# jacke121/p265

Hardware: AMD Instinct MI355X
Metric: reconstructed CTUs/sec (1080p all-intra) + achieved HBM GB/s vs peak (higher is better)
Workload: dtype u8 samples / int16 coefficients (integer)

## Files before the change

p265_amd/csrc/p265r.hip:

```cpp
#include <hip/hip_runtime.h>

#include <algorithm>
#include <array>
#include <chrono>
#include <cstdio>
#include <cstdlib>
#include <ctime>
#include <cstring>
#include <new>
#include <string>
#include <vector>

#include "../../include/p265r.h"
#include "digest.h"
#include "export.h"
#include "export_host.h"
#include "intra.h"
#include "intra_prep.h"
#include "intra_rows.h"
#include "loopfilter.h"
#include "loopfilter16.h"
#include "sao16.h"
#include "residual.h"
#include "coef_expand.h"
// ... 805 lines not shown
    *h2d_bytes = b->h2d_bytes;
    return P265R_OK;
}

int p265r_batch_run(p265r_ctx* ctx, p265r_batch* b) {
    if (!ctx || !b) return P265R_EINVAL;
    HIP_TRY(hipSetDevice(ctx->device));
    hipStream_t s = b->stream;
    Geo g = ctx->geo;
    g.ragged = b->ragged ? 1 : 0;
    p265r_timings tm{};
    hipEvent_t ev[4] = {nullptr, nullptr, nullptr, nullptr};
    if (ctx->timing) {
        for (auto& e : ev) {
            if (!ctx->spare.empty()) { e = ctx->spare.back(); ctx->spare.pop_back(); }
            else HIP_TRY(hipEventCreate(&e));
        }
        HIP_TRY(hipEventRecord(ev[0], s));
    }
    const int bdl = g.bd[0], bdc = g.bd[1];
    const bool recon = !b->recon_input;
    const int skip = b->runs > 0 ? ctx->skip : 0;
    if (ctx->params.scaling_list_enabled && !ctx->d_sf && !b->recon_input) return P265R_ESTATE;
    const uint8_t* sf = ctx->params.scaling_list_enabled ? ctx->d_sf : nullptr;
    ++b->runs;
    ctx->lane_busy |= 1u << b->lane;
    const bool prep = recon && ctx->schedule == 1 && !(skip & 2);
    hipStream_t ps = s;
    const bool big = b->n_pics >= ctx->num_cus;
    const bool sao_aux = P265R_SAO_AUX && !P265R_PHASE_ORDER && !P265R_EARLY_RESIDUAL && ctx->pipeline > 1 && big && prep &&
                         !ctx->timing && ctx->fork_prep == 1 && (b->sao || b->dbk) && !(skip & 4);
    const int fork_prep = big && !sao_aux ? ctx->fork_prep : 0;
    const bool ordered = P265R_PHASE_ORDER && ctx->pipeline > 1 && prep && fork_prep == 1 && !ctx->timing;
    const bool early = !ordered && P265R_EARLY_RESIDUAL && prep && fork_prep == 1 && !ctx->timing && b->intra_done &&
                       !(skip & 1);
    hipEvent_t r_after = ordered ? (ctx->last_intra_valid ? ctx->last_intra_ev : nullptr) : (early ? b->intra_done : nullptr);
    if (ordered && ctx->order_r == 0) r_after = b->intra_done;
    hipStream_t rs = s;
    if ((ordered || early) && r_after) {
        const size_t li = (size_t)b->lane;
        if (ctx->aux2.size() <= li) { ctx->aux2.resize(li + 1, nullptr); ctx->join2_ev.resize(li + 1, nullptr); }
        if (!ctx->aux2[li]) {
            HIP_TRY(hipStreamCreateWithFlags(&ctx->aux2[li], hipStreamNonBlocking));
            HIP_TRY(hipEventCreateWithFlags(&ctx->join2_ev[li], hipEventDisableTiming));
        }
        rs = ctx->aux2[li];
        HIP_TRY(hipStreamWaitEvent(rs, r_after, 0));
        if (b->intra_done && r_after != b->intra_done) HIP_TRY(hipStreamWaitEvent(rs, b->intra_done, 0));
    }
    if (prep && fork_prep) {
        const size_t li = fork_prep == 2 ? 0 : (size_t)b->lane;
        if (ctx->aux.size() <= li) {
            ctx->aux.resize(li + 1, nullptr); ctx->fork_ev.resize(li + 1, nullptr); ctx->join_ev.resize(li + 1, nullptr);
        }
        if (!ctx->aux[li]) {
            if (ctx->stream_prio) {
                int least = 0, greatest = 0;
                HIP_TRY(hipDeviceGetStreamPriorityRange(&least, &greatest));
                HIP_TRY(hipStreamCreateWithPriority(&ctx->aux[li], hipStreamNonBlocking, least));
            } else {
                HIP_TRY(hipStreamCreateWithFlags(&ctx->aux[li], hipStreamNonBlocking));
            }
            HIP_TRY(hipEventCreateWithFlags(&ctx->fork_ev[li], hipEventDisableTiming));
            HIP_TRY(hipEventCreateWithFlags(&ctx->join_ev[li], hipEventDisableTiming));
        }
        ps = ctx->aux[li];
        if ((ordered || early) && r_after) {
            HIP_TRY(hipStreamWaitEvent(ps, r_after, 0));
            if (b->intra_done && r_after != b->intra_done) HIP_TRY(hipStreamWaitEvent(ps, b->intra_done, 0));
        } else {
            HIP_TRY(hipEventRecord(ctx->fork_ev[li], s));
            HIP_TRY(hipStreamWaitEvent(ps, ctx->fork_ev[li], 0));
        }
    }
    auto launch_prep = [&]() -> int {
        Geo gp = g;
        gp.tr_info = (2 * (long long)b->n_pics <= ctx->num_cus || ctx->row_waves == 16) ? 1 : 0;
        intra_prep_kernel<<<dim3(g.wc, g.hc, b->n_pics), 64, ctx->prep_lds, ps>>>(b->d_pics, gp, b->view);
        ++tm.residual_launches;
        if (ps != s) HIP_TRY(hipEventRecord(ctx->join_ev[fork_prep == 2 ? 0 : (size_t)b->lane], ps));
        return P265R_OK;
    };
    if (prep && !ctx->prep_last) { int rc = launch_prep(); if (rc) return rc; }
#define P265R_RES_LAUNCH(K, KSL, blocks, ...)                                                                     \
    do {                                                                                                          \
        if (sf) KSL<<<(blocks), 256, ctx->res_lds, rs>>>(__VA_ARGS__, sf);                                        \
        else K<<<(blocks), 256, ctx->res_lds, rs>>>(__VA_ARGS__, nullptr);                                        \
        ++tm.residual_launches;                                                                                   \
    } while (0)
    if (recon && !(skip & 1) && b->n_jobs[RC_DST4])
        P265R_RES_LAUNCH((residual4_kernel<true, false>), (residual4_kernel<true, true>), (b->n_jobs[RC_DST4] + 255) / 256,
                         b->d_pool, b->d_res, b->d_jobs[RC_DST4], b->n_jobs[RC_DST4], bdl, b->slab[RC_DST4]);
    if (recon && !(skip & 1) && b->n_jobs[RC_DCT4])
        P265R_RES_LAUNCH((residual4_kernel<false, false>), (residual4_kernel<false, true>), (b->n_jobs[RC_DCT4] + 255) / 256,
                         b->d_pool, b->d_res, b->d_jobs[RC_DCT4], b->n_jobs[RC_DCT4], bdc, b->slab[RC_DCT4]);
    if (recon && !(skip & 1) && b->n_jobs[RC_DCT8])
        P265R_RES_LAUNCH((residualN_kernel<3, false>), (residualN_kernel<3, true>), (b->n_jobs[RC_DCT8] + 31) / 32,
                         b->d_pool, b->d_res, b->d_jobs[RC_DCT8], b->n_jobs[RC_DCT8], bdl, bdc, b->slab[RC_DCT8]);
    if (recon && !(skip & 1) && b->n_jobs[RC_DCT16])
        P265R_RES_LAUNCH((residualN_kernel<4, false>), (residualN_kernel<4, true>), (b->n_jobs[RC_DCT16] + 15) / 16,
                         b->d_pool, b->d_res, b->d_jobs[RC_DCT16], b->n_jobs[RC_DCT16], bdl, bdc, b->slab[RC_DCT16]);
    if (recon && !(skip & 1) && b->n_jobs[RC_DCT32])
        P265R_RES_LAUNCH((residualN_kernel<5, false>), (residualN_kernel<5, true>), (b->n_jobs[RC_DCT32] + 7) / 8,
                         b->d_pool, b->d_res, b->d_jobs[RC_DCT32], b->n_jobs[RC_DCT32], bdl, bdc, b->slab[RC_DCT32]);
#undef P265R_RES_LAUNCH
    if (recon && !(skip & 1) && b->n_jobs[RC_TSKIP]) {
        residual_tskip_kernel<<<(b->n_jobs[RC_TSKIP] + 255) / 256, 256, 0, rs>>>(b->d_pool, b->d_res, b->d_jobs[RC_TSKIP], b->n_jobs[RC_TSKIP], bdl, bdc, sf);
        ++tm.residual_launches;
    }
    if (prep && ctx->prep_last) { int rc = launch_prep(); if (rc) return rc; }
    if (prep && ps != s) HIP_TRY(hipStreamWaitEvent(s, ctx->join_ev[fork_prep == 2 ? 0 : (size_t)b->lane], 0));
    if (rs != s) {
        HIP_TRY(hipEventRecord(ctx->join2_ev[(size_t)b->lane], rs));
        HIP_TRY(hipStreamWaitEvent(s, ctx->join2_ev[(size_t)b->lane], 0));
    }
    if (b->dbk) {
        if (g.pel16) dbk_map_kernel<uint16_t><<<dim3(ctx->n_ctus, b->n_pics), 64, 0, s>>>(b->d_pics, g);
        else dbk_map_kernel<uint8_t><<<dim3(ctx->n_ctus, b->n_pics), 64, 0, s>>>(b->d_pics, g);
        ++tm.residual_launches;
    }
    HIP_TRY(hipGetLastError());
    if (ctx->debug_sync) { fprintf(stderr, "[p265r] residual phase enqueued\n"); HIP_TRY(hipStreamSynchronize(s)); fprintf(stderr, "[p265r] residual phase done\n"); }
    if (ctx->timing) HIP_TRY(hipEventRecord(ev[1], s));
    if (recon && ctx->schedule == 1) {
        HIP_TRY(hipMemsetAsync(b->d_err + 64, 0, kRowCuSlots * 16 + (b->d_xg_prog ? sizeof(int) * 2 * ((size_t)g.hc + 1) * b->n_pics : 0), s));
        if (b->sao_pending) { HIP_TRY(hipStreamWaitEvent(s, b->sao_done, 0)); b->sao_pending = false; }
        if (ordered && ctx->last_lf_valid) HIP_TRY(hipStreamWaitEvent(s, ctx->last_lf_ev, 0));
        bool alone = ordered || (ctx->lane_busy & ~(1u << b->lane)) == 0u;
#ifdef P265R_ALONE_PIPE
        alone = alone && ctx->pipeline == 1;
#endif
        int rc = launch_rows(ctx, b, s, alone);
        if (rc) return rc;
        ++tm.intra_launches;
    }
    const int n_steps = (recon && ctx->schedule == 0) ? (g.wc - 1) + 2 * (g.hc - 1) + 1 : 0;
    for (int step = 0; step < n_steps; ++step) {
        const int d = step - (g.wc - 1);
        const int cy_min = d > 0 ? (d + 1) / 2 : 0;
        const int cy_max = std::min(g.hc - 1, step / 2);
        if (cy_max < cy_min) continue;
        dim3 grid(cy_max - cy_min + 1, b->n_pics);
        if (g.pel16) intra_step_kernel<uint16_t><<<grid, 64, 0, s>>>(b->d_pics, b->d_pool, b->d_res, g, step, cy_min);
        else intra_step_kernel<uint8_t><<<grid, 64, 0, s>>>(b->d_pics, b->d_pool, b->d_res, g, step, cy_min);
        ++tm.intra_launches;
    }
    HIP_TRY(hipGetLastError());
    if (recon) {
        if (!b->intra_done) HIP_TRY(hipEventCreateWithFlags(&b->intra_done, hipEventDisableTiming));
        HIP_TRY(hipEventRecord(b->intra_done, s));
        if (!ctx->last_intra_ev) HIP_TRY(hipEventCreateWithFlags(&ctx->last_intra_ev, hipEventDisableTiming));
        HIP_TRY(hipEventRecord(ctx->last_intra_ev, s));
        ctx->last_intra_valid = true;
    }
    if (ctx->debug_sync) { fprintf(stderr, "[p265r] intra phase enqueued\n"); HIP_TRY(hipStreamSynchronize(s)); fprintf(stderr, "[p265r] intra phase done\n"); }
    if (ctx->timing) HIP_TRY(hipEventRecord(ev[2], s));
    const hipStream_t lane_s = s;
    if (sao_aux) {
        const size_t li = (size_t)b->lane;
        if (ctx->aux.size() <= li) {
            ctx->aux.resize(li + 1, nullptr); ctx->fork_ev.resize(li + 1, nullptr); ctx->join_ev.resize(li + 1, nullptr);
        }
        if (!ctx->aux[li]) {
            HIP_TRY(hipStreamCreateWithFlags(&ctx->aux[li], hipStreamNonBlocking));
            HIP_TRY(hipEventCreateWithFlags(&ctx->fork_ev[li], hipEventDisableTiming));
            HIP_TRY(hipEventCreateWithFlags(&ctx->join_ev[li], hipEventDisableTiming));
        }
        if (!b->sao_done) HIP_TRY(hipEventCreateWithFlags(&b->sao_done, hipEventDisableTiming));
        s = ctx->aux[li];
        HIP_TRY(hipStreamWaitEvent(s, b->intra_done, 0));
    }
    if (!(skip & 4)) {
        int rc = launch_loop_filters(ctx, b, g, s, &tm.sao_launches);
        if (rc) return rc;
    }
    if (sao_aux) {
        HIP_TRY(hipEventRecord(b->sao_done, s));
        b->sao_pending = true;
        s = lane_s;
    }
    if (ordered) {
        if (!ctx->last_lf_ev) HIP_TRY(hipEventCreateWithFlags(&ctx->last_lf_ev, hipEventDisableTiming));
        HIP_TRY(hipEventRecord(ctx->last_lf_ev, s));
        ctx->last_lf_valid = true;
    }
    if (ctx->timing) {
        HIP_TRY(hipEventRecord(ev[3], s));
        p265r_ctx::Run run;
        for (int i = 0; i < 4; ++i) run.ev[i] = ev[i];
        run.counts = tm;
// ... 219 lines not shown
    (void)join_sao(b);
    if (ctx->pending == b) ctx->pending = nullptr;
    hipError_t e = b->stream ? hipStreamSynchronize(b->stream) : hipSuccess;
    if (b->intra_done) (void)hipEventDestroy(b->intra_done);
    if (b->sao_done) (void)hipEventDestroy(b->sao_done);
    if (b->d_dig) (void)hipFree(b->d_dig);
    for (void* p : b->exp_idx) (void)hipFree(p);
    if (b->mem) {
        if (!ctx->cache_mem || b->bytes > ctx->cache_bytes) {
            if (ctx->cache_mem) e = hipFree(ctx->cache_mem);
            ctx->cache_mem = b->mem;
            ctx->cache_bytes = b->bytes;
        } else {
            e = hipFree(b->mem);
        }
    }
    delete b;
    return e == hipSuccess ? P265R_OK : hip_fail(e, "hipFree");
}

int p265r_submit(p265r_ctx* ctx, const p265r_picture* pics, int n_pics) {
    if (!ctx) return P265R_EINVAL;
    if (ctx->pending) return P265R_ESTATE;
    p265r_batch* b = nullptr;
    int rc = p265r_batch_upload(ctx, pics, n_pics, &b);
    if (rc) return rc;
    rc = p265r_batch_run(ctx, b);
    if (rc) { p265r_batch_free(ctx, b); return rc; }
    ctx->pending = b;
    ctx->pending_pics.assign(pics, pics + n_pics);
    return P265R_OK;
}

int p265r_wait(p265r_ctx* ctx) {
    if (!ctx) return P265R_EINVAL;
    if (!ctx->pending) return P265R_ESTATE;
    p265r_batch* b = ctx->pending;
    int rc = p265r_batch_download(ctx, b, ctx->pending_pics.data(), (int)ctx->pending_pics.size());
    ctx->pending = nullptr;
    ctx->pending_pics.clear();
    int rc2 = p265r_batch_free(ctx, b);
    return rc ? rc : rc2;
}

int p265r_sync(p265r_ctx* ctx) {
    if (!ctx) return P265R_EINVAL;
    HIP_TRY(hipSetDevice(ctx->device));
    for (hipStream_t st : ctx->lanes) HIP_TRY(hipStreamSynchronize(st));
    for (hipStream_t st : ctx->aux) if (st) HIP_TRY(hipStreamSynchronize(st));
    for (hipStream_t st : ctx->aux2) if (st) HIP_TRY(hipStreamSynchronize(st));
    ctx->lane_busy = 0;
    return P265R_OK;
}

int p265r_set_pipeline(p265r_ctx* ctx, int depth) {
    if (!ctx || depth < 1 || depth > 16) return P265R_EINVAL;
    HIP_TRY(hipSetDevice(ctx->device));
    while ((int)ctx->lanes.size() < depth) {
        hipStream_t st = nullptr;
        HIP_TRY(lane_stream_create(ctx, &st));
        ctx->lanes.push_back(st);
    }
    ctx->pipeline = depth;
    ctx->next_lane = 0;
    return P265R_OK;
}

static const char* hwq_env() {
    const char* v = std::getenv("GPU_MAX_HW_QUEUES");
    return (v && std::strlen(v) < 8 && std::strspn(v, "0123456789") == std::strlen(v)) ? v : "default";
}

int p265r_describe(p265r_ctx* ctx, char* buf, int size) {
    if (!ctx || size < 0 || (size > 0 && !buf)) return P265R_EINVAL;
    const Geo& g = ctx->geo;
    char tmp[2048];
    const int n = snprintf(tmp, sizeof(tmp),
        "{\"schedule\": \"%s\", \"row_waves\": %d, \"row_waves_by_run\": \"%s\", \"lean\": %d, "
        "\"fair\": %d, \"quad\": %d, \"luma_lead\": %d, \"sao_rows\": %d, \"skip\": %d, \"debug_sync\": %d, "
        "\"pipeline\": %d, \"fork_prep\": %d, \"pipe_waves\": %d, \"hw_queues\": \"%s\", \"num_cus\": %d, \"diag_build\": %d, "
        "\"experiments_build\": %d, \"split\": %d, \"last_launch_split\": %d, \"xg\": %d, \"last_launch_xg\": %d, "
        "\"phase_order\": %d, \"early_residual\": %d, \"bit_depth\": %d, \"row_launches\": {\"w12\": %lld, \"w8\": %lld, \"w16_split\": %lld, \"xg\": %lld, \"other\": %lld}, "
        "\"sparse_expand\": \"%s\", \"sparse_expand_stream\": %d, \"last_sparse_expand_ms\": %.4f, "
        "\"env_overrides\": [%s]}",
        ctx->schedule ? "rows" : "steps", ctx->row_waves,
        ctx->row_waves ? "fixed" : (P265R_PHASE_ORDER
                                   ? "batches of >= 1 picture per CU in a pipelined context: W=12, one intra launch at a time "
                                     "(phase order); small batches (< 1 picture per CU: component split, W=16): side by side; "
                                     "otherwise W=12 while no other lane has a run enqueued since the API synchronised it, "
                                     "else pipe_waves"
                                   : "batches of <= CUs / (2 xg) pictures: every luma / chroma chain on xg workgroups of W=4 "
                                     "(cross-group rows, progress and lines in global memory); small batches (< 1 picture per "
                                     "CU: component split, W=16); otherwise W=12 while no other "
                                     "lane has a run enqueued since the API synchronised it, else pipe_waves (W=8, 80 VGPRs: "
                                     "the other lanes' residual / prep / SAO waves fit beside it)"),
        ctx->lean, g.fair, g.quad, ctx->luma_lead, ctx->sao_rows, ctx->skip, ctx->debug_sync ? 1 : 0,
        ctx->pipeline, ctx->fork_prep, ctx->pipe_waves, hwq_env(), ctx->num_cus,
#ifdef P265R_DEBUG_DIAG
        1,
#else
        0,
#endif
        P265R_EXPERIMENTS, ctx->split, ctx->last_split ? 1 : 0, ctx->xg, ctx->last_xg ? 1 : 0, P265R_PHASE_ORDER, P265R_EARLY_RESIDUAL,
        (int)ctx->params.bit_depth_luma, ctx->row_launches[0], ctx->row_launches[1], ctx->row_launches[2], ctx->row_launches[3], ctx->row_launches[4],
        P265R_EXPAND_SCATTER ? "memset + global scatter" : "lds tile", P265R_EXPAND_STREAM, ctx->last_expand_ms,
        ctx->describe.c_str());
    if (n < 0) return P265R_EINVAL;
    if (size > 0) {
        const int k = std::min(n, size - 1);
        std::memcpy(buf, tmp, (size_t)k);
        buf[k] = 0;
    }
    return n;
}

int p265r_set_scaling_factors(p265r_ctx* ctx, const uint8_t* factors, int n_bytes) {
    if (!ctx || !factors || n_bytes != P265R_SCALING_FACTOR_BYTES) return P265R_EINVAL;
    if (!ctx->params.scaling_list_enabled) return P265R_ESTATE;
    for (int i = 0; i < n_bytes; ++i)
        if (factors[i] == 0) return P265R_EINVAL;
    HIP_TRY(hipSetDevice(ctx->device));
    if (int rc = p265r_sync(ctx)) return rc;
    if (!ctx->d_sf) HIP_TRY(hipMalloc(reinterpret_cast<void**>(&ctx->d_sf), P265R_SCALING_FACTOR_BYTES));
    HIP_TRY(hipMemcpy(ctx->d_sf, factors, P265R_SCALING_FACTOR_BYTES, hipMemcpyHostToDevice));
    return P265R_OK;
}

int p265r_set_row_waves(p265r_ctx* ctx, int waves) {
    if (!ctx || (waves != 0 && waves != 8 && waves != 12)) return P265R_EINVAL;
    ctx->row_waves = waves;
    return P265R_OK;
}

int p265r_set_timing(p265r_ctx* ctx, int enable) {
    if (!ctx) return P265R_EINVAL;
    ctx->timing = enable != 0;
    if (enable) {
        for (auto& r : ctx->runs) for (auto& e : r.ev) ctx->spare.push_back(e);
        ctx->runs.clear();
        ctx->have_timing = false;
    }
    return P265R_OK;
}

namespace {
int run_times(const p265r_ctx::Run& r, p265r_timings* t) {
    HIP_TRY(hipEventSynchronize(r.ev[3]));
    float a = 0, b = 0, c = 0, tt = 0;
    HIP_TRY(hipEventElapsedTime(&a, r.ev[0], r.ev[1]));
    HIP_TRY(hipEventElapsedTime(&b, r.ev[1], r.ev[2]));
    HIP_TRY(hipEventElapsedTime(&c, r.ev[2], r.ev[3]));
    HIP_TRY(hipEventElapsedTime(&tt, r.ev[0], r.ev[3]));
    *t = r.counts;
    t->residual_ms = a; t->intra_ms = b; t->sao_ms = c; t->total_ms = tt;
    return P265R_OK;
}
}

int p265r_last_timings(p265r_ctx* ctx, p265r_timings* out) {
    if (!ctx || !out) return P265R_EINVAL;
    if (!ctx->have_timing || ctx->runs.empty()) return P265R_ESTATE;
    HIP_TRY(hipSetDevice(ctx->device));
    return run_times(ctx->runs.back(), out);
}

int p265r_timings_total(p265r_ctx* ctx, p265r_timings* out, int* n_runs) {
    if (!ctx || !out) return P265R_EINVAL;
    if (!ctx->have_timing || ctx->runs.empty()) return P265R_ESTATE;
    HIP_TRY(hipSetDevice(ctx->device));
    p265r_timings sum{};
    for (const auto& r : ctx->runs) {
        p265r_timings t{};
        int rc = run_times(r, &t);
        if (rc) return rc;
        sum.total_ms += t.total_ms; sum.residual_ms += t.residual_ms; sum.intra_ms += t.intra_ms; sum.sao_ms += t.sao_ms;
        sum.intra_launches += t.intra_launches; sum.residual_launches += t.residual_launches;
        sum.sao_launches += t.sao_launches;
    }
    if (n_runs) *n_runs = (int)ctx->runs.size();
    *out = sum;
    return P265R_OK;
}

}
```

p265_amd/csrc/residual.h:

```cpp
#pragma once
#include <hip/hip_runtime.h>
#include <stdint.h>
#include "batch_types.h"
#include "tables.h"

namespace p265r {

#ifndef P265R_RES_NT
#define P265R_RES_NT 0
#endif
typedef unsigned int res_u4 __attribute__((ext_vector_type(4)));
__device__ __forceinline__ void res_store16(int16_t* p, uint32_t a, uint32_t b, uint32_t c, uint32_t d) {
    if constexpr (P265R_RES_NT) __builtin_nontemporal_store(res_u4{a, b, c, d}, reinterpret_cast<res_u4*>(p));
    else *reinterpret_cast<uint4*>(p) = make_uint4(a, b, c, d);
}

__device__ __forceinline__ int clamp16(long long v) {
    return v < -32768 ? -32768 : (v > 32767 ? 32767 : (int)v);
}
__device__ __forceinline__ int clamp16i(int v) {
    return v < -32768 ? -32768 : (v > 32767 ? 32767 : v);
}

struct Dequant {
    int scale, lshift, rshift, rnd;
    __device__ __forceinline__ Dequant(int qp, int bd_shift) {
        const int per = qp / 6;
        scale = 16 * (int)((0x484039332D28ull >> (8 * (qp - 6 * per))) & 0xffu);
        if (per >= bd_shift) { lshift = per - bd_shift; rshift = 0; rnd = 0; }
        else { lshift = 0; rshift = bd_shift - per; rnd = 1 << (rshift - 1); }
        scale <<= lshift;
    }
    __device__ __forceinline__ int operator()(int level) const {
        return clamp16i((__mul24(level, scale) + rnd) >> rshift);
    }
};

__host__ __device__ __forceinline__ int sf_offset(int log2, int c_idx) {
    return log2 == 2 ? 16 * c_idx : (log2 == 3 ? 48 + 64 * c_idx : (log2 == 4 ? 240 + 256 * c_idx : 1008));
}
struct DequantM {
    int ls, per, bds;
    __device__ __forceinline__ DequantM(int qp, int bd_shift) {
        per = qp / 6;
        ls = (int)((0x484039332D28ull >> (8 * (qp - 6 * per))) & 0xffu);
        bds = bd_shift;
    }
    __device__ __forceinline__ int operator()(int level, int m) const {
        const long long v = (long long)(level * m * ls) << per;
        return clamp16((v + (1ll << (bds - 1))) >> bds);
    }
};

template <bool DST>
__device__ __forceinline__ int t4(int j, int i) { return DST ? kDST4[j][i] : kDCT32[j * 8][i]; }

template <bool DST>
__device__ __forceinline__ void inv4(const int (&c)[4], int (&o)[4]) {
    if constexpr (DST) {
        static_assert(kDST4[0][0] == 29 && kDST4[0][1] == 55 && kDST4[1][0] == 74 && kDST4[0][3] == 84, "DST matrix");
        const int a = c[0] + c[2], b = c[2] + c[3], d = c[0] - c[3], e = 74 * c[1];
        o[0] = 29 * a + 55 * b + e;
        o[1] = 55 * d - 29 * b + e;
        o[2] = 74 * (c[0] - c[2] + c[3]);
        o[3] = 55 * a + 29 * d - e;
    } else {
        const int e0 = 64 * (c[0] + c[2]), e1 = 64 * (c[0] - c[2]);
        const int o0 = 83 * c[1] + 36 * c[3], o1 = 36 * c[1] - 83 * c[3];
        o[0] = e0 + o0; o[1] = e1 + o1; o[2] = e1 - o1; o[3] = e0 - o0;
    }
}

template <bool DST, bool SL = false>
__global__ __launch_bounds__(256) void residual4_kernel(const int16_t* __restrict__ pool,
                                                        int16_t* __restrict__ res,
                                                        const ResJob* __restrict__ jobs, int n_jobs,
                                                        int bit_depth, uint32_t slab, const uint8_t* __restrict__ sf) {
    P265R_BW_PRIO_SET();
    const int i = blockIdx.x * blockDim.x + threadIdx.x;
    if (i >= n_jobs) return;
    const ResJob jb = jobs[i];
    const size_t off = (size_t)slab + (size_t)i * 16;
    const int16_t* blk = pool + off;
    int16_t* dst = res + off;
    const uint4 raw0 = *reinterpret_cast<const uint4*>(blk);
    const uint4 raw1 = *reinterpret_cast<const uint4*>(blk + 8);
    const uint32_t w[8] = {raw0.x, raw0.y, raw0.z, raw0.w, raw1.x, raw1.y, raw1.z, raw1.w};
    int d[4][4];
    if constexpr (SL) {
        const DequantM dq(jb.qp, bit_depth + 2 - 5);
        const uint4 mw = *reinterpret_cast<const uint4*>(sf + sf_offset(2, jb.c_idx));
        const uint32_t mv[4] = {mw.x, mw.y, mw.z, mw.w};
#pragma unroll
        for (int k = 0; k < 16; ++k) {
            const int lv = (int)(int16_t)((w[k >> 1] >> ((k & 1) * 16)) & 0xffff);
            d[k >> 2][k & 3] = dq(lv, (int)((mv[k >> 2] >> (8 * (k & 3))) & 0xffu));
        }
    } else {
        const Dequant dq(jb.qp, bit_depth + 2 - 5);
#pragma unroll
        for (int k = 0; k < 16; ++k) {
            const int lv = (int)(int16_t)((w[k >> 1] >> ((k & 1) * 16)) & 0xffff);
            d[k >> 2][k & 3] = dq(lv);
        }
    }
    int g[4][4];
#pragma unroll
    for (int x = 0; x < 4; ++x) {
        const int cin[4] = {d[0][x], d[1][x], d[2][x], d[3][x]};
        int e[4];
        inv4<DST>(cin, e);
#pragma unroll
        for (int y = 0; y < 4; ++y) g[y][x] = clamp16i((e[y] + 64) >> 7);
    }
    const int bd2 = 20 - bit_depth;
    const int rnd2 = 1 << (bd2 - 1);
    uint32_t o[8];
#pragma unroll
    for (int y = 0; y < 4; ++y) {
        int r[4];
        const int rin[4] = {g[y][0], g[y][1], g[y][2], g[y][3]};
        int acc[4];
        inv4<DST>(rin, acc);
#pragma unroll
        for (int x = 0; x < 4; ++x) r[x] = clamp16i((acc[x] + rnd2) >> bd2);
        o[y * 2 + 0] = (uint32_t)(uint16_t)r[0] | ((uint32_t)(uint16_t)r[1] << 16);
        o[y * 2 + 1] = (uint32_t)(uint16_t)r[2] | ((uint32_t)(uint16_t)r[3] << 16);
    }
    res_store16(dst, o[0], o[1], o[2], o[3]);
    res_store16(dst + 8, o[4], o[5], o[6], o[7]);
}

template <int N>
__device__ __forceinline__ void inv_dct_eo(const int (&c)[N], int (&x)[N]) {
    constexpr int H = N / 2;
    constexpr int S = 32 / N;
    int ce[H], ev[H];
#pragma unroll
    for (int k = 0; k < H; ++k) ce[k] = c[2 * k];
    if constexpr (H == 2) {
        ev[0] = kDCT32[0][0] * ce[0] + kDCT32[16][0] * ce[1];
        ev[1] = kDCT32[0][1] * ce[0] + kDCT32[16][1] * ce[1];
    } else {
        inv_dct_eo<H>(ce, ev);
    }
#pragma unroll
    for (int n = 0; n < H; ++n) {
        int od = 0;
#pragma unroll
        for (int j = 0; j < H; ++j) od += kDCT32[(2 * j + 1) * S][n] * c[2 * j + 1];
        x[n] = ev[n] + od;
        x[N - 1 - n] = ev[n] - od;
    }
}

#ifndef P265R_RES_DOT2
#define P265R_RES_DOT2 1
#endif
typedef short res_v2s __attribute__((ext_vector_type(2)));
__device__ __forceinline__ uint32_t pack16(int lo, int hi) {
    return __builtin_amdgcn_perm((uint32_t)hi, (uint32_t)lo, 0x05040100u);
}
template <int N>
__device__ __forceinline__ void inv_dct_d2(const int (&c)[N], int (&x)[N], int rnd64 = 0) {
    constexpr int H = N / 2;
    constexpr int S = 32 / N;
    int ce[H], ev[H];
#pragma unroll
    for (int k = 0; k < H; ++k) ce[k] = c[2 * k];
    if constexpr (H == 2) {
        static_assert(kDCT32[0][0] == 64 && kDCT32[16][0] == 64 && kDCT32[0][1] == 64 && kDCT32[16][1] == -64, "DCT rows 0 / 16");
        ev[0] = 64 * (ce[0] + ce[1] + rnd64);
        ev[1] = 64 * (ce[0] - ce[1] + rnd64);
    } else {
        inv_dct_d2<H>(ce, ev, rnd64);
    }
    if constexpr (H == 2) {
#pragma unroll
        for (int n = 0; n < H; ++n) {
            const int od = kDCT32[S][n] * c[1] + kDCT32[3 * S][n] * c[3];
            x[n] = ev[n] + od;
            x[N - 1 - n] = ev[n] - od;
        }
    } else {
        uint32_t p[H / 2];
#pragma unroll
        for (int j = 0; j < H / 2; ++j) p[j] = pack16(c[4 * j + 1], c[4 * j + 3]);
#pragma unroll
        for (int n = 0; n < H; ++n) {
            int xp = ev[n];
#pragma unroll
            for (int j = 0; j < H / 2; ++j) {
                const uint32_t kk = (uint32_t)(uint16_t)(int16_t)kDCT32[(4 * j + 1) * S][n] |
                                    (uint32_t)(uint16_t)(int16_t)kDCT32[(4 * j + 3) * S][n] << 16;
                xp = __builtin_amdgcn_sdot2(__builtin_bit_cast(res_v2s, p[j]), __builtin_bit_cast(res_v2s, kk), xp, false);
            }
            x[n] = xp;
            x[N - 1 - n] = 2 * ev[n] - xp;
        }
    }
}

template <int LOG2, bool SL = false>
__global__ __launch_bounds__(256) void residualN_kernel(const int16_t* __restrict__ pool,
                                                       int16_t* __restrict__ res,
                                                       const ResJob* __restrict__ jobs, int n_jobs,
                                                       int bit_depth_luma, int bit_depth_chroma, uint32_t slab,
                                                       const uint8_t* __restrict__ sf) {
    P265R_BW_PRIO_SET();
    constexpr int N = 1 << LOG2;
    constexpr int TPB = 256 / N;
    constexpr int S = N + 2;
    __shared__ int16_t tile[TPB][N * S];
    const int local = threadIdx.x / N;
    const int lane = threadIdx.x % N;
    const int job = blockIdx.x * TPB + local;
    const bool active = job < n_jobs;
    int16_t* t = tile[local];
    ResJob jb = active ? jobs[job] : ResJob{0, 0, 0, 0, 0};
    const size_t off = (size_t)slab + (size_t)(active ? job : 0) * (N * N);
    const int16_t* blk = pool + off;
    int16_t* dst = res + off;
    const int bit_depth = jb.c_idx ? bit_depth_chroma : bit_depth_luma;
    if (active && SL) {
        const DequantM dq(jb.qp, bit_depth + LOG2 - 5);
        const uint8_t* mrow = sf + sf_offset(LOG2, jb.c_idx) + lane * N;
#pragma unroll
        for (int v = 0; v < N / 8; ++v) {
            const uint4 raw = *reinterpret_cast<const uint4*>(blk + lane * N + v * 8);
            const uint2 mw = *reinterpret_cast<const uint2*>(mrow + v * 8);
            const uint32_t w[4] = {raw.x, raw.y, raw.z, raw.w};
#pragma unroll
            for (int k = 0; k < 8; ++k) {
                const int lv = (int)(int16_t)((w[k >> 1] >> ((k & 1) * 16)) & 0xffff);
                const int m = (int)((((k < 4) ? mw.x : mw.y) >> (8 * (k & 3))) & 0xffu);
                t[lane * S + v * 8 + k] = (int16_t)dq(lv, m);
            }
        }
    } else if (active) {
        const Dequant dq(jb.qp, bit_depth + LOG2 - 5);
#pragma unroll
        for (int v = 0; v < N / 8; ++v) {
            const uint4 raw = *reinterpret_cast<const uint4*>(blk + lane * N + v * 8);
            const uint32_t w[4] = {raw.x, raw.y, raw.z, raw.w};
#pragma unroll
            for (int k = 0; k < 8; ++k) {
                const int lv = (int)(int16_t)((w[k >> 1] >> ((k & 1) * 16)) & 0xffff);
                t[lane * S + v * 8 + k] = (int16_t)dq(lv);
            }
        }
    }
    __syncthreads();
    if (active) {
        int col[N], e[N];
#pragma unroll
        for (int k = 0; k < N; ++k) col[k] = t[k * S + lane];
#ifdef P265R_RES_NOMATH
#pragma unroll
        for (int k = 0; k < N; ++k) e[k] = col[k] << 7;
#else
        if constexpr (P265R_RES_DOT2) inv_dct_d2<N>(col, e, 1); else inv_dct_eo<N>(col, e);
#endif
#pragma unroll
        for (int y = 0; y < N; ++y) t[y * S + lane] = (int16_t)clamp16i((e[y] + (P265R_RES_DOT2 ? 0 : 64)) >> 7);
    }
    __syncthreads();
    if (active) {
        int row[N], xr[N];
#pragma unroll
        for (int k = 0; k < N; ++k) row[k] = t[lane * S + k];
#ifdef P265R_RES_NOMATH
#pragma unroll
        for (int k = 0; k < N; ++k) xr[k] = row[k];
#else
        if constexpr (P265R_RES_DOT2) inv_dct_d2<N>(row, xr, 1 << (19 - bit_depth - 6)); else inv_dct_eo<N>(row, xr);
#endif
        const int bd2 = 20 - bit_depth;
        const int rnd2 = 1 << (bd2 - 1);
#ifdef P265R_RES_PADV
        {
            uint32_t z = (uint32_t)lane;
#pragma unroll
            for (int q = 0; q < P265R_RES_PADV; ++q) asm volatile("v_add_u32 %0, 1, %0" : "+v"(z));
            asm volatile("" :: "v"(z));
        }
#endif
#pragma unroll
        for (int v = 0; v < N / 8; ++v) {
            uint32_t o[4];
#pragma unroll
            for (int h = 0; h < 4; ++h) {
                int r2[2];
#pragma unroll
                for (int q = 0; q < 2; ++q) {
                    const int x = v * 8 + h * 2 + q;
                    r2[q] = clamp16i((xr[x] + (P265R_RES_DOT2 ? 0 : rnd2)) >> bd2);
                }
                o[h] = (uint32_t)(uint16_t)r2[0] | ((uint32_t)(uint16_t)r2[1] << 16);
            }
            res_store16(dst + lane * N + v * 8, o[0], o[1], o[2], o[3]);
        }
    }
}

__global__ __launch_bounds__(256) void residual_tskip_kernel(const int16_t* __restrict__ pool,
                                                             int16_t* __restrict__ res,
                                                             const ResJob* __restrict__ jobs, int n_jobs,
                                                             int bit_depth_luma, int bit_depth_chroma,
                                                             const uint8_t* __restrict__ sf) {
    const int i = blockIdx.x * blockDim.x + threadIdx.x;
    if (i >= n_jobs) return;
    const ResJob jb = jobs[i];
    const int bd = jb.c_idx ? bit_depth_chroma : bit_depth_luma;
    const Dequant dq(jb.qp, bd + jb.log2 - 5);
    const DequantM dqm(jb.qp, bd + jb.log2 - 5);
    const uint8_t* m = sf ? sf + sf_offset(jb.log2, jb.c_idx) : nullptr;
    const int ts = 5 + jb.log2;
    const int bd2 = 20 - bd;
    const int n2 = 1 << (2 * jb.log2);
    const int16_t* blk = pool + jb.off;
    int16_t* dst = res + jb.off;
    for (int k = 0; k < n2; ++k) {
        const long long r = (long long)(m ? dqm(blk[k], m[k]) : dq(blk[k])) << ts;
        dst[k] = (int16_t)clamp16((r + (1 << (bd2 - 1))) >> bd2);
    }
}

}
```

p265_amd/recon.py:

```python
import ctypes
from dataclasses import dataclass

import numpy as np

from . import _lib
from . import records as R


def _params_c(p):
    c = _lib.Params()
    for name, _ in _lib.Params._fields_:
        if name == "reserved":
            continue
        setattr(c, name, int(p[name]))
    return c


def sparsify(pic):
    lib = _lib.load()
    tbs_in = np.ascontiguousarray(pic.tbs, R.TB_DTYPE)
    coef = np.ascontiguousarray(pic.coef, np.int16)
    c = _lib.PictureC()
    c.tbs = tbs_in.ctypes.data if len(tbs_in) else None
    c.n_tbs = len(tbs_in)
    c.coef = coef.ctypes.data if len(coef) else None
    c.n_coef = len(coef)
    n_nz, n_raw = ctypes.c_uint64(0), ctypes.c_uint64(0)
    _lib.check(lib.p265r_sparsify(ctypes.byref(c), None, None, 0, ctypes.byref(n_nz), None, 0, ctypes.byref(n_raw)),
               "p265r_sparsify")
    tbs = np.zeros(len(tbs_in), R.TB_DTYPE)
    nz = np.zeros(n_nz.value, np.uint32)
    raw = np.zeros(n_raw.value, np.int16)
    _lib.check(lib.p265r_sparsify(ctypes.byref(c), tbs.ctypes.data, nz.ctypes.data, len(nz), ctypes.byref(n_nz),
                                  raw.ctypes.data, len(raw), ctypes.byref(n_raw)), "p265r_sparsify")
    return R.SparsePicture(ctus=pic.ctus, tbs=tbs, nz=nz, coef=raw, nofilter=pic.nofilter, size=pic.size,
                           recon_input=pic.recon_input, meta=dict(pic.meta))


def plane_shapes(params):
    w, h = int(params["pic_width"]), int(params["pic_height"])
    return [(h, w), (h // 2, w // 2), (h // 2, w // 2)]


class DecodedPicture:

    def __init__(self, planes, recon):
        self.planes, self.recon = planes, recon

    @staticmethod
    def _at(planes, x, y, c_idx):
        sub = 1 if c_idx else 0
        return int(planes[c_idx][y >> sub, x >> sub])

    def get_reconstructed_sample(self, x, y, c_idx):
        return self._at(self.recon, x, y, c_idx)

    def get_output_sample(self, x, y, c_idx):
        return self._at(self.planes, x, y, c_idx)


_FORMATS = {"planar": _lib.FMT_PLANAR, "semiplanar": _lib.FMT_SEMIPLANAR, "rgb_planar": _lib.FMT_RGB_PLANAR,
            "rgb_packed": _lib.FMT_RGB_PACKED}
_SAMPLES = {"native": _lib.SMP_NATIVE, "msb16": _lib.SMP_MSB16, "u8": _lib.SMP_U8, "f16": _lib.SMP_F16,
            "f32": _lib.SMP_F32}
_MATRICES = {"bt601": _lib.MAT_BT601, "bt709": _lib.MAT_BT709, "bt2020": _lib.MAT_BT2020}
_UPSAMPLES = {"nearest": _lib.UP_NEAREST, "bilinear": _lib.UP_BILINEAR}


@dataclass(frozen=True)
class ExportSpec:
    format: object = "planar"
    sample: object = "native"
    matrix: object = "bt709"
    full_range: bool = False
    upsample: object = "nearest"
    crop: tuple = (0, 0, 0, 0)
    pitch_align: int = 1

    @staticmethod
    def named(name, **kw):
        table = {"i420": ("planar", "native"), "nv12": ("semiplanar", "native"), "p010": ("semiplanar", "msb16"),
                 "rgb24": ("rgb_packed", "u8"), "rgb-planar-f16": ("rgb_planar", "f16")}
        if name not in table:
            raise ValueError("unknown output format %r" % (name,))
        return ExportSpec(format=table[name][0], sample=table[name][1], **kw)

    def desc(self):
        def enum(v, names, what):
            if isinstance(v, str):
# ... 422 lines not shown
```

Before: 52.08 million.

## Add configurable residual block size, per-TB unrolling with prefetch, and wave-level sync

Restructures the residual kernels so each thread or TB-group processes U transform blocks in a loop, prefetching the next block's coefficients and job while computing the current one. Block size becomes a compile-time knob, and a 64-thread block can replace __syncthreads with a wave-level sync. Out-of-range jobs are clamped to the last valid job and computed with stores masked, instead of returning early. The defaults keep block 256 and unroll 1, so the default path mostly keeps the old launch geometry, with a little extra redundant work on tail groups.

```diff
diff --git a/p265_amd/csrc/p265r.hip b/p265_amd/csrc/p265r.hip
--- a/p265_amd/csrc/p265r.hip
+++ b/p265_amd/csrc/p265r.hip
@@ -911,30 +911,27 @@
         return P265R_OK;
     };
     if (prep && !ctx->prep_last) { int rc = launch_prep(); if (rc) return rc; }
-#define P265R_RES_LAUNCH(K, KSL, blocks, ...)                                                                     \
+#define P265R_RES_LAUNCH(K, KSL, cls, log2, ...)                                                                  \
     do {                                                                                                          \
-        if (sf) KSL<<<(blocks), 256, ctx->res_lds, rs>>>(__VA_ARGS__, sf);                                        \
-        else K<<<(blocks), 256, ctx->res_lds, rs>>>(__VA_ARGS__, nullptr);                                        \
+        const int n_tb = b->n_jobs[cls];                                                                          \
+        const int blocks = (n_tb + res_block_tbs(log2) - 1) / res_block_tbs(log2);      \
+        if (sf) KSL<<<blocks, kResBlock, ctx->res_lds, rs>>>(b->d_pool, b->d_res, b->d_jobs[cls], n_tb, __VA_ARGS__, b->slab[cls], sf);      \
+        else K<<<blocks, kResBlock, ctx->res_lds, rs>>>(b->d_pool, b->d_res, b->d_jobs[cls], n_tb, __VA_ARGS__, b->slab[cls], nullptr);      \
         ++tm.residual_launches;                                                                                   \
     } while (0)
     if (recon && !(skip & 1) && b->n_jobs[RC_DST4])
-        P265R_RES_LAUNCH((residual4_kernel<true, false>), (residual4_kernel<true, true>), (b->n_jobs[RC_DST4] + 255) / 256,
-                         b->d_pool, b->d_res, b->d_jobs[RC_DST4], b->n_jobs[RC_DST4], bdl, b->slab[RC_DST4]);
+        P265R_RES_LAUNCH((residual4_kernel<true, false>), (residual4_kernel<true, true>), RC_DST4, 2, bdl);
     if (recon && !(skip & 1) && b->n_jobs[RC_DCT4])
-        P265R_RES_LAUNCH((residual4_kernel<false, false>), (residual4_kernel<false, true>), (b->n_jobs[RC_DCT4] + 255) / 256,
-                         b->d_pool, b->d_res, b->d_jobs[RC_DCT4], b->n_jobs[RC_DCT4], bdc, b->slab[RC_DCT4]);
+        P265R_RES_LAUNCH((residual4_kernel<false, false>), (residual4_kernel<false, true>), RC_DCT4, 2, bdc);
     if (recon && !(skip & 1) && b->n_jobs[RC_DCT8])
-        P265R_RES_LAUNCH((residualN_kernel<3, false>), (residualN_kernel<3, true>), (b->n_jobs[RC_DCT8] + 31) / 32,
-                         b->d_pool, b->d_res, b->d_jobs[RC_DCT8], b->n_jobs[RC_DCT8], bdl, bdc, b->slab[RC_DCT8]);
+        P265R_RES_LAUNCH((residualN_kernel<3, false>), (residualN_kernel<3, true>), RC_DCT8, 3, bdl, bdc);
     if (recon && !(skip & 1) && b->n_jobs[RC_DCT16])
-        P265R_RES_LAUNCH((residualN_kernel<4, false>), (residualN_kernel<4, true>), (b->n_jobs[RC_DCT16] + 15) / 16,
-                         b->d_pool, b->d_res, b->d_jobs[RC_DCT16], b->n_jobs[RC_DCT16], bdl, bdc, b->slab[RC_DCT16]);
+        P265R_RES_LAUNCH((residualN_kernel<4, false>), (residualN_kernel<4, true>), RC_DCT16, 4, bdl, bdc);
     if (recon && !(skip & 1) && b->n_jobs[RC_DCT32])
-        P265R_RES_LAUNCH((residualN_kernel<5, false>), (residualN_kernel<5, true>), (b->n_jobs[RC_DCT32] + 7) / 8,
-                         b->d_pool, b->d_res, b->d_jobs[RC_DCT32], b->n_jobs[RC_DCT32], bdl, bdc, b->slab[RC_DCT32]);
+        P265R_RES_LAUNCH((residualN_kernel<5, false>), (residualN_kernel<5, true>), RC_DCT32, 5, bdl, bdc);
 #undef P265R_RES_LAUNCH
     if (recon && !(skip & 1) && b->n_jobs[RC_TSKIP]) {
-        residual_tskip_kernel<<<(b->n_jobs[RC_TSKIP] + 255) / 256, 256, 0, rs>>>(b->d_pool, b->d_res, b->d_jobs[RC_TSKIP], b->n_jobs[RC_TSKIP], bdl, bdc, sf);
+        residual_tskip_kernel<<<(b->n_jobs[RC_TSKIP] + kResBlock - 1) / kResBlock, kResBlock, 0, rs>>>(b->d_pool, b->d_res, b->d_jobs[RC_TSKIP], b->n_jobs[RC_TSKIP], bdl, bdc, sf);
         ++tm.residual_launches;
     }
     if (prep && ctx->prep_last) { int rc = launch_prep(); if (rc) return rc; }
@@ -1320,6 +1317,7 @@
         "\"experiments_build\": %d, \"split\": %d, \"last_launch_split\": %d, \"xg\": %d, \"last_launch_xg\": %d, "
         "\"phase_order\": %d, \"early_residual\": %d, \"bit_depth\": %d, \"row_launches\": {\"w12\": %lld, \"w8\": %lld, \"w16_split\": %lld, \"xg\": %lld, \"other\": %lld}, "
         "\"sparse_expand\": \"%s\", \"sparse_expand_stream\": %d, \"last_sparse_expand_ms\": %.4f, "
+        "\"residual\": {\"block\": %d, \"wave_sync\": %d, \"unroll4\": %d, \"unroll\": %d, \"unroll32\": %d}, "
         "\"env_overrides\": [%s]}",
         ctx->schedule ? "rows" : "steps", ctx->row_waves,
         ctx->row_waves ? "fixed" : (P265R_PHASE_ORDER
@@ -1342,6 +1340,7 @@
         P265R_EXPERIMENTS, ctx->split, ctx->last_split ? 1 : 0, ctx->xg, ctx->last_xg ? 1 : 0, P265R_PHASE_ORDER, P265R_EARLY_RESIDUAL,
         (int)ctx->params.bit_depth_luma, ctx->row_launches[0], ctx->row_launches[1], ctx->row_launches[2], ctx->row_launches[3], ctx->row_launches[4],
         P265R_EXPAND_SCATTER ? "memset + global scatter" : "lds tile", P265R_EXPAND_STREAM, ctx->last_expand_ms,
+        kResBlock, P265R_RES_WAVESYNC ? 1 : 0, res_unroll(2), res_unroll(3), res_unroll(5),
         ctx->describe.c_str());
     if (n < 0) return P265R_EINVAL;
     if (size > 0) {
diff --git a/p265_amd/csrc/residual.h b/p265_amd/csrc/residual.h
--- a/p265_amd/csrc/residual.h
+++ b/p265_amd/csrc/residual.h
@@ -2,9 +2,37 @@
 #include <hip/hip_runtime.h>
 #include <stdint.h>
 #include "batch_types.h"
+#include "intra_rows.h"
 #include "tables.h"
 
 namespace p265r {
+
+#ifndef P265R_RES_BLOCK
+#define P265R_RES_BLOCK 256
+#endif
+#ifndef P265R_RES_WAVESYNC
+#define P265R_RES_WAVESYNC (P265R_RES_BLOCK == 64)
+#endif
+#ifndef P265R_RES_UNROLL
+#define P265R_RES_UNROLL 1
+#endif
+#ifndef P265R_RES_UNROLL4
+#define P265R_RES_UNROLL4 P265R_RES_UNROLL
+#endif
+#ifndef P265R_RES_UNROLL32
+#define P265R_RES_UNROLL32 1
+#endif
+constexpr int kWave = 64;
+constexpr int kResBlock = P265R_RES_BLOCK;
+static_assert(kResBlock == 64 || kResBlock == 128 || kResBlock == 256, "whole waves, at most 256 threads");
+__host__ __device__ constexpr int res_unroll(int log2) {
+    return log2 == 5 ? P265R_RES_UNROLL32 : (log2 == 2 ? P265R_RES_UNROLL4 : P265R_RES_UNROLL);
+}
+static_assert(res_unroll(2) >= 1 && res_unroll(2) <= 4 && res_unroll(3) >= 1 && res_unroll(3) <= 4 &&
+              res_unroll(5) >= 1 && res_unroll(5) <= 4, "U");
+__host__ __device__ constexpr int res_block_tbs(int log2) {
+    return (log2 == 2 ? kResBlock : kResBlock >> log2) * res_unroll(log2);
+}
 
 #ifndef P265R_RES_NT
 #define P265R_RES_NT 0
@@ -71,21 +99,18 @@
     }
 }
 
-template <bool DST, bool SL = false>
-__global__ __launch_bounds__(256) void residual4_kernel(const int16_t* __restrict__ pool,
-                                                        int16_t* __restrict__ res,
-                                                        const ResJob* __restrict__ jobs, int n_jobs,
-                                                        int bit_depth, uint32_t slab, const uint8_t* __restrict__ sf) {
-    P265R_BW_PRIO_SET();
-    const int i = blockIdx.x * blockDim.x + threadIdx.x;
-    if (i >= n_jobs) return;
-    const ResJob jb = jobs[i];
-    const size_t off = (size_t)slab + (size_t)i * 16;
-    const int16_t* blk = pool + off;
-    int16_t* dst = res + off;
-    const uint4 raw0 = *reinterpret_cast<const uint4*>(blk);
-    const uint4 raw1 = *reinterpret_cast<const uint4*>(blk + 8);
-    const uint32_t w[8] = {raw0.x, raw0.y, raw0.z, raw0.w, raw1.x, raw1.y, raw1.z, raw1.w};
+struct Res4In { uint4 raw0, raw1; ResJob jb; };
+__device__ __forceinline__ Res4In res4_load(const int16_t* pool, const ResJob* jobs,
+                                            uint32_t slab, int i) {
+    const int16_t* blk = pool + ((size_t)slab + (size_t)i * 16);
+    return Res4In{*reinterpret_cast<const uint4*>(blk), *reinterpret_cast<const uint4*>(blk + 8), jobs[i]};
+}
+
+template <bool DST, bool SL>
+__device__ __forceinline__ void res4_tb(const Res4In& in, bool active, int16_t* dst, int bit_depth,
+                                        const uint8_t* __restrict__ sf) {
+    const ResJob jb = in.jb;
+    const uint32_t w[8] = {in.raw0.x, in.raw0.y, in.raw0.z, in.raw0.w, in.raw1.x, in.raw1.y, in.raw1.z, in.raw1.w};
     int d[4][4];
     if constexpr (SL) {
         const DequantM dq(jb.qp, bit_depth + 2 - 5);
@@ -127,8 +152,29 @@
         o[y * 2 + 0] = (uint32_t)(uint16_t)r[0] | ((uint32_t)(uint16_t)r[1] << 16);
         o[y * 2 + 1] = (uint32_t)(uint16_t)r[2] | ((uint32_t)(uint16_t)r[3] << 16);
     }
-    res_store16(dst, o[0], o[1], o[2], o[3]);
-    res_store16(dst + 8, o[4], o[5], o[6], o[7]);
+    if (active) {
+        res_store16(dst, o[0], o[1], o[2], o[3]);
+        res_store16(dst + 8, o[4], o[5], o[6], o[7]);
+    }
+}
+
+template <bool DST, bool SL = false>
+__global__ __launch_bounds__(kResBlock) void residual4_kernel(const int16_t* pool, int16_t* res,
+                                                              const ResJob* jobs, int n_jobs,
+                                                              int bit_depth, uint32_t slab, const uint8_t* __restrict__ sf) {
+    P265R_BW_PRIO_SET();
+    constexpr int U = res_unroll(2);
+    int i = blockIdx.x * (kResBlock * U) + threadIdx.x;
+    if (i >= n_jobs) return;
+    Res4In cur = res4_load(pool, jobs, slab, i);
+#pragma unroll
+    for (int u = 0; u < U; ++u) {
+        Res4In nxt = cur;
+        if (u + 1 < U) nxt = res4_load(pool, jobs, slab, min(i + kResBlock, n_jobs - 1));
+        res4_tb<DST, SL>(cur, i < n_jobs, res + ((size_t)slab + (size_t)i * 16), bit_depth, sf);
+        cur = nxt;
+        i += kResBlock;
+    }
 }
 
 template <int N>
@@ -201,33 +247,35 @@
     }
 }
 
-template <int LOG2, bool SL = false>
-__global__ __launch_bounds__(256) void residualN_kernel(const int16_t* __restrict__ pool,
-                                                       int16_t* __restrict__ res,
-                                                       const ResJob* __restrict__ jobs, int n_jobs,
-                                                       int bit_depth_luma, int bit_depth_chroma, uint32_t slab,
-                                                       const uint8_t* __restrict__ sf) {
-    P265R_BW_PRIO_SET();
+__device__ __forceinline__ void res_sync() {
+    if constexpr (P265R_RES_WAVESYNC) wave_sync(); else __syncthreads();
+}
+
+template <int N> struct ResNIn { uint4 raw[N / 8]; ResJob jb; };
+template <int N>
+__device__ __forceinline__ void resN_load(ResNIn<N>& in, const int16_t* __restrict__ pool,
+                                          const ResJob* __restrict__ jobs, uint32_t slab, int job, int lane) {
+    const int16_t* row = pool + ((size_t)slab + (size_t)job * (N * N)) + lane * N;
+#pragma unroll
+    for (int v = 0; v < N / 8; ++v) in.raw[v] = *reinterpret_cast<const uint4*>(row + v * 8);
+    in.jb = jobs[job];
+}
+
+template <int LOG2, bool SL>
+__device__ __forceinline__ void resN_set(const ResNIn<(1 << LOG2)>& in, bool active, int job, int lane, int16_t* t,
+                                         int16_t* __restrict__ res, int bit_depth_luma, int bit_depth_chroma,
+                                         uint32_t slab, const uint8_t* __restrict__ sf) {
     constexpr int N = 1 << LOG2;
-    constexpr int TPB = 256 / N;
     constexpr int S = N + 2;
-    __shared__ int16_t tile[TPB][N * S];
-    const int local = threadIdx.x / N;
-    const int lane = threadIdx.x % N;
-    const int job = blockIdx.x * TPB + local;
-    const bool active = job < n_jobs;
-    int16_t* t = tile[local];
-    ResJob jb = active ? jobs[job] : ResJob{0, 0, 0, 0, 0};
-    const size_t off = (size_t)slab + (size_t)(active ? job : 0) * (N * N);
-    const int16_t* blk = pool + off;
-    int16_t* dst = res + off;
+    const ResJob jb = in.jb;
+    int16_t* dst = res + ((size_t)slab + (size_t)job * (N * N));
     const int bit_depth = jb.c_idx ? bit_depth_chroma : bit_depth_luma;
-    if (active && SL) {
+    if constexpr (SL) {
         const DequantM dq(jb.qp, bit_depth + LOG2 - 5);
         const uint8_t* mrow = sf + sf_offset(LOG2, jb.c_idx) + lane * N;
 #pragma unroll
         for (int v = 0; v < N / 8; ++v) {
-            const uint4 raw = *reinterpret_cast<const uint4*>(blk + lane * N + v * 8);
+            const uint4 raw = in.raw[v];
             const uint2 mw = *reinterpret_cast<const uint2*>(mrow + v * 8);
             const uint32_t w[4] = {raw.x, raw.y, raw.z, raw.w};
 #pragma unroll
@@ -237,11 +285,11 @@
                 t[lane * S + v * 8 + k] = (int16_t)dq(lv, m);
             }
         }
-    } else if (active) {
+    } else {
         const Dequant dq(jb.qp, bit_depth + LOG2 - 5);
 #pragma unroll
         for (int v = 0; v < N / 8; ++v) {
-            const uint4 raw = *reinterpret_cast<const uint4*>(blk + lane * N + v * 8);
+            const uint4 raw = in.raw[v];
             const uint32_t w[4] = {raw.x, raw.y, raw.z, raw.w};
 #pragma unroll
             for (int k = 0; k < 8; ++k) {
@@ -250,8 +298,8 @@
             }
         }
     }
-    __syncthreads();
-    if (active) {
+    res_sync();
+    {
         int col[N], e[N];
 #pragma unroll
         for (int k = 0; k < N; ++k) col[k] = t[k * S + lane];
@@ -264,8 +312,8 @@
 #pragma unroll
         for (int y = 0; y < N; ++y) t[y * S + lane] = (int16_t)clamp16i((e[y] + (P265R_RES_DOT2 ? 0 : 64)) >> 7);
     }
-    __syncthreads();
-    if (active) {
+    res_sync();
+    {
         int row[N], xr[N];
 #pragma unroll
         for (int k = 0; k < N; ++k) row[k] = t[lane * S + k];
@@ -298,12 +346,40 @@
                 }
                 o[h] = (uint32_t)(uint16_t)r2[0] | ((uint32_t)(uint16_t)r2[1] << 16);
             }
-            res_store16(dst + lane * N + v * 8, o[0], o[1], o[2], o[3]);
-        }
-    }
-}
-
-__global__ __launch_bounds__(256) void residual_tskip_kernel(const int16_t* __restrict__ pool,
+            if (active) res_store16(dst + lane * N + v * 8, o[0], o[1], o[2], o[3]);
+        }
+    }
+}
+
+template <int LOG2, bool SL = false>
+__global__ __launch_bounds__(kResBlock) void residualN_kernel(const int16_t* __restrict__ pool,
+                                                             int16_t* __restrict__ res,
+                                                             const ResJob* __restrict__ jobs, int n_jobs,
+                                                             int bit_depth_luma, int bit_depth_chroma, uint32_t slab,
+                                                             const uint8_t* __restrict__ sf) {
+    P265R_BW_PRIO_SET();
+    constexpr int N = 1 << LOG2;
+    constexpr int TPB = kResBlock / N;
+    constexpr int U = res_unroll(LOG2);
+    static_assert(kWave % N == 0 && kResBlock % kWave == 0, "a TB's N threads are consecutive lanes of one wave");
+    __shared__ int16_t tile[TPB][N * (N + 2)];
+    const int local = threadIdx.x / N;
+    const int lane = threadIdx.x % N;
+    int16_t* t = tile[local];
+    int job = blockIdx.x * (TPB * U) + local;
+    ResNIn<N> cur;
+    resN_load<N>(cur, pool, jobs, slab, min(job, n_jobs - 1), lane);
+#pragma unroll
+    for (int u = 0; u < U; ++u) {
+        ResNIn<N> nxt = cur;
+        if (u + 1 < U) resN_load<N>(nxt, pool, jobs, slab, min(job + TPB, n_jobs - 1), lane);
+        resN_set<LOG2, SL>(cur, job < n_jobs, job, lane, t, res, bit_depth_luma, bit_depth_chroma, slab, sf);
+        cur = nxt;
+        job += TPB;
+    }
+}
+
+__global__ __launch_bounds__(kResBlock) void residual_tskip_kernel(const int16_t* __restrict__ pool,
                                                              int16_t* __restrict__ res,
                                                              const ResJob* __restrict__ jobs, int n_jobs,
                                                              int bit_depth_luma, int bit_depth_chroma,
diff --git a/p265_amd/recon.py b/p265_amd/recon.py
--- a/p265_amd/recon.py
+++ b/p265_amd/recon.py
@@ -5,6 +5,11 @@
 
 from . import _lib
 from . import records as R
+
+
+RES_WAVE = 64
+RES_SET_TBS = {"dst4": RES_WAVE, "dct4": RES_WAVE, "dct8": RES_WAVE // 8, "dct16": RES_WAVE // 16,
+               "dct32": RES_WAVE // 32}
 
 
 def _params_c(p):
```

Result: no change. 52.21 million, median of 3 (+0.2%).
